# Nuttoty/Structured_Light_for_3D_Model_Replication

Hardware: AMD Instinct MI355X
Metric: decoded+triangulated px/s (higher is better)
Workload: dtype u8+f64

## Files before the change

structured_light_for_3d_model_replication_amd/csrc/slgpu.hip:

```cpp
#include <hip/hip_runtime.h>

#include <math.h>
#include <stdint.h>
#include <stdlib.h>
#include <string.h>

#include <stdio.h>

#include <algorithm>
#include <cmath>
#include <initializer_list>
#include <string>
#include <type_traits>
#include <thread>
#include <vector>

#include <dlfcn.h>
#include <errno.h>
#include <fcntl.h>
#include <sys/stat.h>
#include <unistd.h>

#include <chrono>
#include <condition_variable>
#include <memory>
#include <mutex>

#include "rccl/rccl.h"
#include "slgpu.h"

#pragma clang fp contract(off)

namespace {

constexpr int kThreads = 256;
constexpr int kWaves = kThreads / 64;
constexpr int kPx = 16;
constexpr int kChunk = 64 * kPx;
constexpr int kChunkNib = kChunk / 4;
constexpr int kRing = 40;
constexpr int kLoadAux = 2;
constexpr int kRecAux = 16;
constexpr int kMapAux = 2;
typedef unsigned v4u __attribute__((ext_vector_type(4)));
typedef unsigned v2u __attribute__((ext_vector_type(2)));
__device__ __forceinline__ uint4 ld_side16(const void* p) { return *reinterpret_cast<const uint4*>(p); }
__device__ __forceinline__ uint2 ld_side8(const void* p) { return *reinterpret_cast<const uint2*>(p); }
__device__ __forceinline__ uint32_t ld_side4(const void* p) { return *reinterpret_cast<const uint32_t*>(p); }

constexpr int M_MAPS = 1;
constexpr int M_CODES = 2;
constexpr int M_XYZ64 = 4;
constexpr int M_FROMMAPS = 8;
constexpr int M_NC = 16;
constexpr int M_ROWS = 32;
constexpr int M_HIST = 64;
constexpr int M_FAST32 = 128;
constexpr int M_PLANE_RSRC = 512;
constexpr int M_TEX = 2048;
constexpr int M_VERIFY = 4096;
constexpr int M_DECIDE = 256;
constexpr float kFastKappa = 16.0f;

constexpr int kSlot = 272;
constexpr int kSlotArrive = 257;
constexpr int kHistRep = 8;
constexpr int kHistStride = kHistRep + 1;
constexpr int kMaxWp = 32768;
constexpr int64_t kMaxChunks = 1 << 16;
constexpr int kRecSlot = 1536;

struct ViewStats {
  int thr_white;
  int thr_contrast;
  float noise_floor;
  float dynamic_range;
  unsigned pad[12];
};
static_assert(sizeof(ViewStats) % 64 == 0, "ViewStats keeps 64-B alignment");

struct Params {
  const uint8_t* stack;
  int64_t stack_vs;
  int view_bytes;
  const uint8_t* tex;
  int64_t tex_vs;
  const int32_t* in_col;
  const uint8_t* in_mask;
  int64_t HW;
  int H, W;
  uint32_t w_magic;
  int w_shift;
  int n_views;
  int cpv;
  int64_t n_chunks;
  int nc, nr, kc, kr;
  int mode;
  int Wp;
  const double4* planes;
  const float4* planes32;
  const double* xn;
  const double* yn;
  const float* xn32;
  const float* yn32;
  float fast_thr;
  int xy_safe;
  int xy_calc;
  double cx, cy, fx, fy;
  double rfx, rfy;
  const double* nc_rays;
  double o0, o1, o2;
  const double* poses;
  uint16_t* codes;
  int rec12;
  int rec_blk;
  uint8_t* ptnib;
  int32_t* col_out;
  int32_t* row_out;
  uint8_t* mask_out;
  void* xyz;
  uint8_t* bgr;
  int64_t out_cap;
  int64_t* view_offsets;
  ViewStats* stats;
  unsigned long long* masked;
  unsigned* hist;
  const int64_t* base_in;
  int* chunk_counts;
  int* block_sums;
  int bs_atomic;
  int decode_dyn;
  unsigned* super_base;
  unsigned* super_par;
  int sb_shift;
  int rerun;
  int cloud_gx;
  const uint8_t* pre_stack;
  int64_t pre_vs;
  unsigned* pre_hist;
  int pre_views;
  int pre_bpv;
};


__device__ __forceinline__ int64_t rec_slot(const Params& p, int view, int civ) {
  return (static_cast<int64_t>(civ >> 2) * p.n_views + view) * 4 + (civ & 3);
}

__device__ __forceinline__ uint4 ld16(const uint8_t* p, int n, bool vec) {
  if (vec) return *reinterpret_cast<const uint4*>(p);
  uint32_t w[4] = {0u, 0u, 0u, 0u};
#pragma unroll
  for (int i = 0; i < 16; ++i)
    if (i < n) w[i >> 2] |= static_cast<uint32_t>(p[i]) << (8 * (i & 3));
  return make_uint4(w[0], w[1], w[2], w[3]);
}

__device__ __forceinline__ uint32_t word(const uint4& q, int i) {
  return i == 0 ? q.x : i == 1 ? q.y : i == 2 ? q.z : q.w;
}

__device__ __forceinline__ uint32_t byte_of(const uint4& q, int i) {
// ... 175 lines not shown
  return fabs((pl.x * r0 + pl.y * r1) + pl.z * r2) > 1e-6;
}

__device__ __forceinline__ bool has_point(const Params& p, int mode, const float4& f, int c, float x, float y,
                                          float z, float inv, int u, int v, int64_t q) {
  const float a = fabsf((f.x * x + f.y * y + f.z * z) * inv);
  const float S = (fabsf(f.x * x) + fabsf(f.y * y) + fabsf(f.z * z)) * inv;
  const float B = S * 3.814697265625e-06f + 9.5367431640625e-13f;
  if (a > 1e-6f + B) return true;
  if (a < 1e-6f - B) return false;
  return has_point_f64(p.planes, p.xn, p.yn, (mode & M_NC) ? p.nc_rays : nullptr, p.HW, c, u, v, q);
}


__global__ __launch_bounds__(256) void k_xy_check(const double* xn, int W, const double* yn, int H, double cx,
                                                  double cy, double fx, double fy, int* bad) {
  const int i = static_cast<int>(blockIdx.x) * 256 + static_cast<int>(threadIdx.x);
  bool diff = false;
  if (i < W) diff = __double_as_longlong(xy_of(i, cx, fx)) != __double_as_longlong(xn[i]);
  else if (i < W + H) diff = __double_as_longlong(xy_of(i - W, cy, fy)) != __double_as_longlong(yn[i - W]);
  if (diff) *bad = 1;
}

constexpr int kHistRepl = 8;
constexpr int kHistView = kHistRepl * kSlot;

__device__ __forceinline__ void stats_pass(const uint8_t* vb, int64_t HW, int64_t blk, int64_t nblk, unsigned* gh,
                                           unsigned* s_hist, int* s_max) {
  const int tid = threadIdx.x;
  const int lane = tid & 63;
  const int wid = __builtin_amdgcn_readfirstlane(tid >> 6);
  for (int i = tid; i < 256 * kHistStride; i += kThreads) s_hist[i] = 0u;
  __syncthreads();
  unsigned* hrow = s_hist + (lane & (kHistRep - 1));
  int mx = -1024;
  const int64_t n16 = HW / 16;
  for (int64_t i = blk * kThreads + tid; i < n16; i += nblk * kThreads) {
    const uint4 wq = ld_side16(vb + 16 * i);
    const uint4 bq = ld_side16(vb + HW + 16 * i);
#pragma unroll
    for (int k = 0; k < 16; ++k) {
      const int bk = static_cast<int>(byte_of(bq, k));
      atomicAdd(hrow + bk * kHistStride, 1u);
      mx = max(mx, static_cast<int>(byte_of(wq, k)) - bk);
    }
  }
#pragma unroll
  for (int d = 32; d > 0; d >>= 1) mx = max(mx, __shfl_xor(mx, d, 64));
  if (lane == 0) s_max[wid] = mx;
  __syncthreads();
  gh += (blk % kHistRepl) * kSlot;
  unsigned cnt = 0u;
  const unsigned* row = s_hist + tid * kHistStride;
#pragma unroll
  for (int r = 0; r < kHistRep; ++r) cnt += row[r];
  if (cnt) atomicAdd(gh + tid, cnt);
  if (tid == 0) {
    int m = s_max[0];
#pragma unroll
    for (int w = 1; w < kWaves; ++w) m = max(m, s_max[w]);
    if (m > -1024) atomicMax(gh + 256, static_cast<unsigned>(m + 1024));
  }
}

__global__ __launch_bounds__(kThreads) void k_stats(Params p) {
  __shared__ unsigned s_hist[256 * kHistStride];
  __shared__ int s_max[kWaves];
  const int view = blockIdx.y;
  stats_pass(p.stack + view * p.stack_vs, p.HW, blockIdx.x, gridDim.x, p.hist + static_cast<int64_t>(view) * kHistView,
             s_hist, s_max);
}

__device__ __forceinline__ void pre_stats_block(const Params& p, int64_t sx, int64_t nsx, unsigned* s_hist,
                                                int* s_max) {
  const int64_t sblk = static_cast<int64_t>(blockIdx.y) * nsx + sx;
  const int64_t total = static_cast<int64_t>(p.pre_views) * p.pre_bpv;
  if (sblk < total) {
    const int pv = static_cast<int>(sblk / p.pre_bpv);
    stats_pass(p.pre_stack + pv * p.pre_vs, p.HW, sblk - static_cast<int64_t>(pv) * p.pre_bpv, p.pre_bpv,
               p.pre_hist + static_cast<int64_t>(pv) * kHistView, s_hist, s_max);
  }
}

__device__ __forceinline__ Thresholds view_thresholds(const Params& p, int view, int lane) {
  uint4 b4 = make_uint4(0u, 0u, 0u, 0u);
  unsigned hmax = 0u;
  const unsigned* h = p.hist + static_cast<int64_t>(view) * kHistView;
#pragma unroll
  for (int r = 0; r < kHistRepl; ++r) {
    const uint4 t = reinterpret_cast<const uint4*>(h + r * kSlot)[lane];
    b4.x += t.x;
    b4.y += t.y;
    b4.z += t.z;
    b4.w += t.w;
    hmax = max(hmax, h[r * kSlot + 256]);
  }
  return thresholds_from_bins(b4, hmax, p.HW, lane);
}

template <int S>
__device__ __forceinline__ bool arrive_last(unsigned* ctr, unsigned id, unsigned readers) {
  const unsigned cls = id & (S - 1);
  const unsigned n_cls = (readers - cls + S - 1) / S;
  if (atomicAdd(ctr + 1 + cls, 1u) + 1u != n_cls) return false;
  return atomicAdd(ctr, 1u) + 1u == min(readers, static_cast<unsigned>(S));
}

__device__ __forceinline__ void hist_release(unsigned* h, int words, unsigned id, unsigned readers, int lane,
                                             uint32_t dep0, uint32_t dep1) {
  asm volatile("" ::"v"(dep0), "v"(dep1) : "memory");
  unsigned last = 0u;
  if (lane == 0) last = arrive_last<8>(h + kSlotArrive, id, readers) ? 1u : 0u;
  if (__shfl(static_cast<int>(last), 0, 64)) {
    uint4* h4 = reinterpret_cast<uint4*>(h);
    for (int i = lane; i < words / 4; i += 64) h4[i] = make_uint4(0u, 0u, 0u, 0u);
  }
}

__device__ __forceinline__ uint32_t mask4(uint32_t w, uint32_t b, uint32_t tw2, uint32_t tc2, uint32_t* bytes) {
  const uint32_t we = w & 0x00ff00ffu, wo = (w >> 8) & 0x00ff00ffu;
  const uint32_t be = b & 0x00ff00ffu, bo = (b >> 8) & 0x00ff00ffu;
  const uint32_t me = ((we | 0x80008000u) - tw2) & (((we + 0x00100010u) | 0x80008000u) - (be + tc2));
  const uint32_t mo = ((wo | 0x80008000u) - tw2) & (((wo + 0x00100010u) | 0x80008000u) - (bo + tc2));
  const uint32_t y = ((me >> 15) & 0x00010001u) | ((mo >> 7) & 0x01000100u);
  *bytes = y;
  return (y & 1u) | ((y >> 7) & 2u) | ((y >> 14) & 4u) | ((y >> 21) & 8u);
}

constexpr int kDecPl = 2048, kDecX = 4096, kDecY = 4096;
constexpr int kDecPlWords = kDecPl * 4;
constexpr int kBsSlots = 64;
constexpr int kSuperCap = 4096;
constexpr int kSuperWords = 2 * kSuperCap + 4;

__device__ __forceinline__ unsigned* super_produce(const Params& p) {
  const unsigned sel = p.super_par[0] & 1u;
  if (!p.rerun && blockIdx.x == 0 && blockIdx.y == 0) {
    unsigned* other = p.super_base + (sel ^ 1u) * kSuperCap;
    for (int i = threadIdx.x; i < kSuperCap; i += kThreads) other[i] = 0u;
    if (threadIdx.x == 0) p.super_par[1] = sel;
  }
  return p.super_base + sel * kSuperCap;
}
__device__ __forceinline__ const unsigned* super_consume(const Params& p, int bx) {
  const unsigned sel = p.super_par[1] & 1u;
  if (!p.rerun && bx == 0 && blockIdx.y == 0 && threadIdx.x == 0) p.super_par[0] = sel ^ 1u;
  return p.super_base + sel * kSuperCap;
}
constexpr int kDecodeLds = (kDecPlWords + kDecX) * 4;
static_assert(kDecodeLds >= 256 * kHistStride * 4, "the decode LDS holds the histogram replicas too");

constexpr int kDecodePerCu = 3;
template <int KC, int KR, int MODE, int VEC>
__global__ __launch_bounds__(kThreads, 3) void k_decode(Params p) {
  const int mode = MODE >= 0 ? MODE : p.mode;
  const int kc = KC >= 0 ? KC : p.kc;
  const int krr = (mode & M_ROWS) ? (KR >= 0 ? KR : p.kr) : 0;
  const int nc = p.nc, nr = p.nr;
  const bool vec = VEC > 0;
  const bool hist = (mode & M_HIST) && !(mode & M_DECIDE);

  __shared__ __attribute__((aligned(16))) unsigned s_lds[kDecodeLds / 4];
  __shared__ int s_max[kWaves];
  __shared__ int s_cnt[2][kWaves];
  __shared__ unsigned s_bsum[kBsSlots];
  __shared__ uint32_t s_thr[2];
  __shared__ unsigned s_mcount;
  __shared__ int s_next[2];
  __shared__ uint4 s_mapst[(MODE < 0 || (MODE & M_MAPS)) ? 64 * kWaves : 1];
  unsigned* s_hist = s_lds;
  float4* s_pl = reinterpret_cast<float4*>(s_lds);
  float* s_xn = reinterpret_cast<float*>(s_lds) + kDecPlWords;
  const bool decide = (mode & M_DECIDE) != 0;
  const int tid = threadIdx.x;
  const int lane = tid & 63;
  const int wid = __builtin_amdgcn_readfirstlane(tid >> 6);
  const int view = blockIdx.y;
  const int64_t HW = p.HW;
  const int gx = static_cast<int>(gridDim.x);
  if (decide) {
    if (tid < kBsSlots) s_bsum[tid] = 0u;
    if (tid == 0) s_mcount = 0u;
    if ((mode & M_HIST) && wid == 0) {
      const Thresholds t = view_thresholds(p, view, lane);
      if (lane == 0) {
        s_thr[0] = static_cast<uint32_t>(t.white + 1) * 0x00010001u;
        s_thr[1] = static_cast<uint32_t>(t.contrast + 17) * 0x00010001u;
        if (blockIdx.x == 0) {
          p.stats[view].thr_white = t.white;
          p.stats[view].thr_contrast = t.contrast;
          p.stats[view].noise_floor = t.noise_floor;
          p.stats[view].dynamic_range = t.dynamic_range;
        }
      }
    }
    if (mode & M_CODES) {
      const int wp_t = min(p.Wp, kDecPl), w_t = min(p.W, kDecX);
      typedef __attribute__((address_space(3))) void* lds_ptr_t;
      for (int i = wid; i * 64 < wp_t; i += kWaves)
        __builtin_amdgcn_global_load_lds(p.planes32 + min(i * 64 + lane, wp_t - 1), (lds_ptr_t)(s_pl + i * 64), 16, 0, 0);
      for (int i = wid; i * 256 < w_t; i += kWaves)
        __builtin_amdgcn_global_load_lds(p.xn32 + min(i * 256 + 4 * lane, w_t - 4), (lds_ptr_t)(s_xn + i * 256), 16, 0, 0);
    }
  }
  uint32_t tw2 = static_cast<uint32_t>(40 + 1) * 0x00010001u;
  uint32_t tc2 = static_cast<uint32_t>(10 + 17) * 0x00010001u;
  int it = 0;

  if (hist) {
    for (int i = tid; i < 256 * kHistStride; i += kThreads) s_hist[i] = 0u;
    __syncthreads();
  }

  const int ngroups = (p.cpv + kWaves - 1) / kWaves;
  int mx_acc = -1024;
  const bool dyn = p.decode_dyn && decide && (mode & M_CODES) && !p.bs_atomic;
  unsigned* const sup = (decide && (mode & M_CODES)) ? super_produce(p) : nullptr;
  unsigned* const dyn_ctr = sup + (kSuperCap - 1 - view);
  for (int cg = blockIdx.x; cg < ngroups;) {
  unsigned dyn_next = 0u;
  if (dyn && tid == 0) dyn_next = atomicAdd(dyn_ctr, 1u);
  const int civ = cg * kWaves + wid;
  const bool live = civ < p.cpv;
  const int64_t px0 = static_cast<int64_t>(civ) * kChunk + lane * kPx;
  const int n_px = live ? static_cast<int>(min<int64_t>(max<int64_t>(HW - px0, 0), kPx)) : 0;
  const int64_t pxl = n_px > 0 ? px0 : 0;
  const int64_t o = view * HW + px0;

  const float ys_early = (decide && (mode & M_CODES) && n_px > 0) ? p.yn32[row_of(p, static_cast<int>(px0))] : 0.0f;
  uint32_t col[kPx];
  uint32_t pt_rec = 0xffffu;
  uint4 wq = make_uint4(0u, 0u, 0u, 0u), bq = wq;
  uint32_t rA[4] = {0, 0, 0, 0}, rB[4] = {0, 0, 0, 0};
  const int rBn = krr > 8 ? krr - 8 : 0;
  const int rSh = nr - krr;
  if (mode & M_FROMMAPS) {
    const int64_t ol = view * HW + pxl;
    if (vec) {
      const int4* cm = reinterpret_cast<const int4*>(p.in_col + ol);
#pragma unroll
      for (int i = 0; i < 4; ++i) {
        const int4 v = cm[i];
        col[4 * i] = static_cast<uint32_t>(max(v.x, 0));
        col[4 * i + 1] = static_cast<uint32_t>(max(v.y, 0));
        col[4 * i + 2] = static_cast<uint32_t>(max(v.z, 0));
        col[4 * i + 3] = static_cast<uint32_t>(max(v.w, 0));
      }
    } else {
#pragma unroll
      for (int k = 0; k < kPx; ++k) col[k] = k < n_px ? static_cast<uint32_t>(max(p.in_col[ol + k], 0)) : 0u;
    }
  } else {
    const uint8_t* vbase = p.stack + view * p.stack_vs;
    const int voff = static_cast<int>(pxl);
    const __amdgpu_buffer_rsrc_t rs_view =
        __builtin_amdgcn_make_buffer_rsrc(const_cast<uint8_t*>(vbase), 0, p.view_bytes, 0x00020000);
    auto ldp = [&](int plane) -> uint4 {
      if (vec && !(mode & M_PLANE_RSRC)) {
        const auto v = __builtin_amdgcn_raw_buffer_load_b128(rs_view, voff, plane * static_cast<int>(HW), kLoadAux);
        return make_uint4(v[0], v[1], v[2], v[3]);
      }
      if (vec) {
        const __amdgpu_buffer_rsrc_t rs = __builtin_amdgcn_make_buffer_rsrc(
            const_cast<uint8_t*>(vbase) + static_cast<int64_t>(plane) * HW, 0, static_cast<int>(HW), 0x00020000);
        const auto v = __builtin_amdgcn_raw_buffer_load_b128(rs, voff, 0, kLoadAux);
        return make_uint4(v[0], v[1], v[2], v[3]);
      }
      return ld16(vbase + pxl + static_cast<int64_t>(plane) * HW, n_px, false);
    };
    wq = ldp(0);
    bq = ldp(1);
    const int npl = 2 * (kc + krr);
    uint32_t cA[4] = {0, 0, 0, 0}, cB[4] = {0, 0, 0, 0};
    auto consume = [&](const uint4& P, const uint4& I, int pair) {
      auto ins = [](uint32_t acc, uint32_t g) { return ((acc >> 1) & 0x7f7f7f7fu) | (g & 0x80808080u); };
      uint32_t g[4];
#pragma unroll
      for (int w = 0; w < 4; ++w) g[w] = gt_bit7(word(P, w), word(I, w));
#pragma unroll
      for (int w = 0; w < 4; ++w) {
        if (pair < kc) {
          if (pair < 8) cA[w] = ins(cA[w], g[w]);
          else cB[w] = ins(cB[w], g[w]);
        } else if (pair - kc < 8) {
          rA[w] = ins(rA[w], g[w]);
        } else {
          rB[w] = ins(rB[w], g[w]);
        }
      }
// ... 32 lines not shown
            const uint4 I = ring[j + 1];
            if (pl + R < npl) {
              ring[j] = ldp(2 + pl + R);
              ring[j + 1] = ldp(3 + pl + R);
            }
            consume(P, I, pl >> 1);
          }
        }
      }
    }
    auto to_binary = [](uint32_t (&A)[4], uint32_t (&B)[4], int k) {
      const int kA = k < 8 ? k : 8, kB = k - kA;
#pragma unroll
      for (int w = 0; w < 4; ++w) {
        A[w] = gray_to_binary_bytes(__builtin_bitreverse32(A[w]), kA);
        B[w] = kB > 0 ? gray_to_binary_bytes(__builtin_bitreverse32(B[w]) ^ ((A[w] & 0x01010101u) << (kB - 1)), kB)
                      : 0u;
      }
    };
    const int cBn = kc > 8 ? kc - 8 : 0;
    const int cSh = nc - kc;
    to_binary(cA, cB, kc);
#pragma unroll
    for (int q = 0; q < kPx; ++q) {
      const int w = q >> 2, sft = 8 * (3 - (q & 3));
      col[q] = (((cA[w] >> sft) & 0xffu) << cBn) | ((cB[w] >> sft) & 0xffu);
    }
    if (cSh > 0) {
#pragma unroll
      for (int q = 0; q < kPx; ++q) {
        const uint32_t lo = col[q] & 1u;
        col[q] = (col[q] << cSh) | ((lo << cSh) - lo);
      }
    }
    if (mode & M_ROWS) to_binary(rA, rB, krr);
  }
  auto row_code = [&](int w, int e) -> uint32_t {
    const int sft = 8 * (3 - e);
    uint32_t v = (((rA[w] >> sft) & 0xffu) << rBn) | ((rB[w] >> sft) & 0xffu);
    if (rSh > 0) {
      const uint32_t lo = v & 1u;
      v = (v << rSh) | ((lo << rSh) - lo);
    }
    return v;
  };
  if (mode & M_MAPS) {
    if (vec && live) {
      uint4* const stg = s_mapst + 64 * wid;
      const int64_t cbase = view * HW + static_cast<int64_t>(civ) * kChunk;
#pragma unroll
      for (int m = 0; m < 2; ++m) {
        const __amdgpu_buffer_rsrc_t rd = __builtin_amdgcn_make_buffer_rsrc(
            (m == 0 ? p.col_out : p.row_out) + cbase, 0,
            static_cast<int>(4 * min<int64_t>(kChunk, HW - static_cast<int64_t>(civ) * kChunk)), 0x00020000);
#pragma unroll
        for (int j = 0; j < 4; ++j) {
          if ((lane >> 4) == j && n_px == kPx) {
            const int u = lane & 15;
#pragma unroll
            for (int q = 0; q < 4; ++q) {
              uint32_t v4[4];
#pragma unroll
              for (int e = 0; e < 4; ++e) v4[e] = m == 0 ? col[4 * q + e] : row_code(q, e);
              stg[4 * u + q] = make_uint4(v4[0], v4[1], v4[2], v4[3]);
            }
          }
          __builtin_amdgcn_wave_barrier();
          const uint4 v = stg[lane];
          __builtin_amdgcn_wave_barrier();
          __builtin_amdgcn_raw_buffer_store_b128(v4u{v.x, v.y, v.z, v.w}, rd, 1024 * j + 16 * lane, 0, kMapAux);
        }
      }
    } else if (!vec) {
#pragma unroll
      for (int k = 0; k < kPx; ++k) {
        if (k < n_px) {
          __builtin_nontemporal_store(static_cast<int32_t>(col[k]), p.col_out + o + k);
          __builtin_nontemporal_store(static_cast<int32_t>(row_code(k >> 2, k & 3)), p.row_out + o + k);
        }
      }
    }
  }
  if (decide) {
    if (it == 0) {
      __syncthreads();
      if (mode & M_HIST) {
        tw2 = __builtin_amdgcn_readfirstlane(s_thr[0]);
        tc2 = __builtin_amdgcn_readfirstlane(s_thr[1]);
      }
    }
    uint32_t ok = 0u, mb[4];
#pragma unroll
    for (int w = 0; w < 4; ++w) ok |= mask4(word(wq, w), word(bq, w), tw2, tc2, &mb[w]) << (4 * w);
    if (n_px != kPx) ok = 0u;
    if (p.masked) {
      const int mc = wave_sum_dpp(__popc(ok));
      if (lane == 0 && mc) atomicAdd(&s_mcount, static_cast<unsigned>(mc));
    }
    if ((mode & M_MAPS) && n_px == kPx)
      __builtin_nontemporal_store(v4u{mb[0], mb[1], mb[2], mb[3]}, reinterpret_cast<v4u*>(p.mask_out + o));
    uint32_t pt = 0u;
    if ((mode & M_CODES) && ok) {
      const int px0i = static_cast<int>(px0);
      const int v = row_of(p, px0i), u0 = px0i - v * p.W;
      float4 pf[kPx];
#pragma unroll
      for (int k = 0; k < kPx; ++k) pf[k] = s_pl[min(col[k], static_cast<uint32_t>(p.Wp - 1))];
      float xs[kPx];
#pragma unroll
      for (int q4 = 0; q4 < 4; ++q4) {
        const float4 x4 = reinterpret_cast<const float4*>(s_xn + u0)[q4];
        xs[4 * q4] = x4.x;
        xs[4 * q4 + 1] = x4.y;
        xs[4 * q4 + 2] = x4.z;
        xs[4 * q4 + 3] = x4.w;
      }
      const float ys = ys_early;
      uint32_t todo = ok;
      if (!(mode & M_NC)) {
#pragma unroll
        for (int k = 0; k < kPx; ++k) {
          const float a = fabsf(__builtin_fmaf(pf[k].x, xs[k], __builtin_fmaf(pf[k].y, ys, pf[k].z)));
          if (a > p.fast_thr) pt |= 1u << k;
        }
        pt &= ok;
        todo &= ~pt;
      }
#pragma unroll
      for (int k = 0; k < kPx; ++k) {
        if (!((todo >> k) & 1u)) continue;
        const int c = static_cast<int>(min(col[k], static_cast<uint32_t>(p.Wp - 1)));
        const int64_t q = px0 + k;
        float x, y, z, inv;
        if (mode & M_NC) {
          x = static_cast<float>(p.nc_rays[q]);
          y = static_cast<float>(p.nc_rays[HW + q]);
          z = static_cast<float>(p.nc_rays[2 * HW + q]);
          inv = 1.0f;
        } else {
          x = xs[k];
          y = ys;
          z = 1.0f;
          inv = __frsqrt_rn(x * x + y * y + 1.0f);
        }
        if (has_point(p, mode, pf[k], c, x, y, z, inv, u0 + k, v, q)) pt |= 1u << k;
      }
    }
    if (mode & M_CODES) {
      const int64_t gci = static_cast<int64_t>(view) * p.cpv + civ;
      pt_rec = pt;
      const int cnt = wave_sum_dpp(__popc(pt));
      if (lane == 0) {
        if (live) p.chunk_counts[gci] = cnt;
        const unsigned mine = live ? static_cast<unsigned>(cnt) : 0u;
        if (p.bs_atomic) {
          const unsigned old = atomicAdd(&s_bsum[it], (1u << 16) | mine);
          if ((old >> 16) == kWaves - 1) {
            const int64_t blk = static_cast<int64_t>(view) * ngroups + cg;
            const unsigned t = (old & 0xffffu) + mine;
            p.block_sums[blk] = static_cast<int>(t);
            if (t) atomicAdd(sup + (blk >> p.sb_shift), t);
          }
        } else {
          s_cnt[it & 1][wid] = static_cast<int>(mine);
        }
      }
    }
  }
  if (hist) {
    unsigned* hrow = s_hist + (lane & (kHistRep - 1));
    int mx = -1024;
#pragma unroll
    for (int k = 0; k < kPx; ++k) {
      if (k < n_px) {
        const int bk = static_cast<int>(byte_of(bq, k));
        atomicAdd(hrow + bk * kHistStride, 1u);
        mx = max(mx, static_cast<int>(byte_of(wq, k)) - bk);
      }
    }
    mx_acc = max(mx_acc, mx);
  }

  if (mode & M_CODES) {
    uint32_t rec[kPx / 2];
#pragma unroll
    for (int i = 0; i < kPx / 2; ++i)
      rec[i] = min(col[2 * i], static_cast<uint32_t>(p.Wp - 1)) |
               (min(col[2 * i + 1], static_cast<uint32_t>(p.Wp - 1)) << 16);
    if (decide) {
      const bool blk = !(mode & M_MAPS);
      if (n_px == kPx) {
        uint32_t rw[6];
        uint32_t* ro = blk ? rw : reinterpret_cast<uint32_t*>(reinterpret_cast<uint8_t*>(p.codes) + 3 * o / 2);
#pragma unroll
        for (int h = 0; h < 2; ++h) {
          const uint32_t* r = rec + 4 * h;
          auto cd = [&](int k, uint32_t c) { return ((pt_rec >> (8 * h + k)) & 1u) ? c : 0xfffu; };
          const uint32_t c0 = cd(0, r[0] & 0xffffu), c1 = cd(1, r[0] >> 16), c2 = cd(2, r[1] & 0xffffu);
          const uint32_t c3 = cd(3, r[1] >> 16), c4 = cd(4, r[2] & 0xffffu), c5 = cd(5, r[2] >> 16);
          const uint32_t c6 = cd(6, r[3] & 0xffffu), c7 = cd(7, r[3] >> 16);
          ro[3 * h] = c0 | (c1 << 12) | (c2 << 24);
          ro[3 * h + 1] = (c2 >> 8) | (c3 << 4) | (c4 << 16) | (c5 << 28);
          ro[3 * h + 2] = (c5 >> 4) | (c6 << 8) | (c7 << 20);
        }
        if (blk) {
          const __amdgpu_buffer_rsrc_t rs = __builtin_amdgcn_make_buffer_rsrc(
              reinterpret_cast<uint8_t*>(p.codes) + kRecSlot * rec_slot(p, view, civ), 0, kRecSlot, 0x00020000);
          __builtin_amdgcn_raw_buffer_store_b128(v4u{rw[0], rw[1], rw[2], rw[3]}, rs, 16 * lane, 0, kRecAux);
          __builtin_amdgcn_raw_buffer_store_b64(v2u{rw[4], rw[5]}, rs, 1024 + 8 * lane, 0, kRecAux);
        }
      }
    } else if (vec) {
      if (n_px == kPx) {
        uint4* ro = reinterpret_cast<uint4*>(p.codes + o);
        ro[0] = make_uint4(rec[0], rec[1], rec[2], rec[3]);
        ro[1] = make_uint4(rec[4], rec[5], rec[6], rec[7]);
      }
    } else {
#pragma unroll
      for (int k = 0; k < kPx; ++k)
        if (k < n_px) p.codes[o + k] = static_cast<uint16_t>(rec[k >> 1] >> (16 * (k & 1)));
    }
  }
  if (decide && (mode & M_CODES) && !p.bs_atomic) {
    if (dyn && tid == 0) s_next[it & 1] = static_cast<int>(dyn_next) + gx;
    __syncthreads();
    if (tid == 0) {
      int t = 0;
#pragma unroll
      for (int w = 0; w < kWaves; ++w) t += s_cnt[it & 1][w];
      const int64_t blk = static_cast<int64_t>(view) * ngroups + cg;
      p.block_sums[blk] = t;
      if (t) atomicAdd(sup + (blk >> p.sb_shift), static_cast<unsigned>(t));
    }
  }
  cg = dyn ? s_next[it & 1] : cg + gx;
  ++it;
  }

  if (decide && p.masked) {
    __syncthreads();
    if (tid == 0 && s_mcount) atomicAdd(p.masked + view, static_cast<unsigned long long>(s_mcount));
  }
  if (decide && (mode & M_HIST) && !p.rerun && wid == 0)
    hist_release(p.hist + static_cast<int64_t>(view) * kHistView, kHistView, blockIdx.x, gx, lane, tw2, tc2);

  if (hist) {
#pragma unroll
    for (int d = 32; d > 0; d >>= 1) mx_acc = max(mx_acc, __shfl_xor(mx_acc, d, 64));
    if (lane == 0) s_max[wid] = mx_acc;
    __syncthreads();
    unsigned* gh = p.hist + view * kSlot;
    unsigned cnt = 0u;
    const unsigned* row = s_hist + tid * kHistStride;
#pragma unroll
    for (int r = 0; r < kHistRep; ++r) cnt += row[r];
    if (cnt) atomicAdd(gh + tid, cnt);
    if (tid == 0) {
      int m = s_max[0];
#pragma unroll
      for (int w = 1; w < kWaves; ++w) m = max(m, s_max[w]);
      if (m > -1024) atomicMax(gh + 256, static_cast<unsigned>(m + 1024));
    }
  }
}

template <int VEC>
__device__ __forceinline__ int count_chunk(const Params& p, int64_t gc, int view, int civ, int lane, bool live,
                                           int* masked) {
  const int mode = p.mode;
  const bool vec = VEC > 0;
  const int HW = static_cast<int>(p.HW);
  const int cpx = civ * kChunk;
  const int W = p.W;
  const bool codes = (mode & M_CODES) != 0;
  const bool nc = (mode & M_NC) != 0;
  const uint8_t* vstack = p.stack + view * p.stack_vs;
  const uint16_t* vcodes = codes ? p.codes + static_cast<int64_t>(view) * HW : nullptr;

  uint4 hb = make_uint4(0u, 0u, 0u, 0u);
  unsigned hmax = 0u;
  const bool adaptive = (mode & M_HIST) != 0;
  if (adaptive) {
    const unsigned* h = p.hist + view * kSlot;
    hb = reinterpret_cast<const uint4*>(h)[lane];
    hmax = h[256];
  }
  uint32_t wv[4], bv[4];
  uint32_t rc[4][2];
  const int px_hi = vec ? HW - 4 : HW - 1;
#pragma unroll
  for (int s = 0; s < 4; ++s) {
    const int px = min(cpx + 256 * s + 4 * lane, px_hi);
    if (mode & M_FROMMAPS) {
      wv[s] = bv[s] = 0u;
    } else if (vec) {
      wv[s] = ld_side4(vstack + px);
      bv[s] = ld_side4(vstack + HW + px);
    } else {
      uint32_t a = 0u, b = 0u;
#pragma unroll
      for (int e = 0; e < 4; ++e) {
        const int q = min(px + e, HW - 1);
        a |= static_cast<uint32_t>(vstack[q]) << (8 * e);
        b |= static_cast<uint32_t>(vstack[HW + q]) << (8 * e);
      }
      wv[s] = a;
      bv[s] = b;
    }
    if (codes) {
      if (vec) {
        const uint2 r = ld_side8(vcodes + px);
        rc[s][0] = r.x;
        rc[s][1] = r.y;
      } else {
        rc[s][0] = vcodes[min(px, HW - 1)] | (static_cast<uint32_t>(vcodes[min(px + 1, HW - 1)]) << 16);
        rc[s][1] = vcodes[min(px + 2, HW - 1)] | (static_cast<uint32_t>(vcodes[min(px + 3, HW - 1)]) << 16);
      }
    }
  }
  uint32_t mk[4] = {0u, 0u, 0u, 0u};
  if (mode & M_FROMMAPS) {
    const uint8_t* vm = p.in_mask + static_cast<int64_t>(view) * HW;
#pragma unroll
    for (int s = 0; s < 4; ++s) {
      const int px = cpx + 256 * s + 4 * lane;
#pragma unroll
      for (int e = 0; e < 4; ++e) mk[s] |= (px + e < HW && vm[px + e] != 0) ? (1u << e) : 0u;
    }
// ... 986 lines not shown
}

__global__ __launch_bounds__(256) void k_zero(unsigned* p, int64_t n) {
  for (int64_t i = static_cast<int64_t>(blockIdx.x) * 256 + threadIdx.x; i < n; i += 256ll * gridDim.x) p[i] = 0u;
}
int zero_async(sl_ctx* c, void* p, int64_t words, hipStream_t s) {
  if (words <= 0) return SL_OK;
  const unsigned blocks = static_cast<unsigned>(std::min<int64_t>((words + 255) / 256, 1024));
  hipLaunchKernelGGL(k_zero, dim3(blocks), dim3(256), 0, s, static_cast<unsigned*>(p), words);
  HIP_TRY(c, hipGetLastError());
  return SL_OK;
}
int capture_of(sl_ctx* c, hipStream_t s, unsigned long long* out) {
  hipStreamCaptureStatus st = hipStreamCaptureStatusNone;
  unsigned long long id = 0;
  HIP_TRY(c, hipStreamGetCaptureInfo(s, &st, &id));
  *out = st == hipStreamCaptureStatusActive ? id + 1 : 0;
  return SL_OK;
}

int launch_groups(sl_ctx* c, const Params& p0, bool vec, int decode_mode, int count_mode, int cloud_mode,
                  hipStream_t s, PreArms arms) {
  const bool decide = (decode_mode & M_DECIDE) != 0;
  const bool codes = (decode_mode & M_CODES) != 0;
  const int64_t cpv = p0.cpv;
  const int vpg = static_cast<int>(std::max<int64_t>(1, kMaxChunks / cpv));
  const int n_groups = static_cast<int>((p0.n_views + vpg - 1) / vpg);
  const bool adaptive = (decode_mode & M_HIST) != 0;
  const bool pre_run = arms.decl && cloud_mode >= 0 && vec;
  bool hist_fresh = false;
  int r = ensure_scratch(c, std::min(vpg, p0.n_views), p0.HW, codes, pre_run ? std::min(vpg, c->decl_views) : 0,
                         &hist_fresh, s, true);
  if (r) return r;
  r = grow(c, &c->d_stats, &c->cap_stats, p0.n_views, s, true);
  if (r) return r;
  unsigned long long cap_id = 0;
  r = capture_of(c, s, &cap_id);
  if (r) return r;
  const int nv0 = std::min(vpg, p0.n_views);
  const bool pre_use = arms.armed && !hist_fresh && decide && adaptive && p0.stack == c->pre_stack &&
                       p0.stack_vs == c->pre_vs && nv0 == c->pre_views && p0.HW == c->pre_hw &&
                       c->pre_capture == cap_id;
  const bool pre_groups = decide && adaptive && n_groups > 1 && cloud_mode >= 0 && vec;
  const int dom = cap_id ? 1 : 0;
  unsigned* const hbuf = c->d_hist[dom];
  int64_t& hist_dirty = c->hist_dirty[dom];
  if (dom == 1 && c->cap_domain != cap_id) {
    c->cap_domain = cap_id;
    hist_dirty = c->cap_hist;
  }
  if (c->super_dirty) {
    r = zero_async(c, c->d_super, kSuperWords, s);
    if (r) return r;
  }
  c->super_dirty = false;
  if (!pre_use && hist_dirty > 0) {
    r = zero_async(c, hbuf, hist_dirty, s);
    if (r) return r;
  }
  if (!pre_use) hist_dirty = 0;
  auto pre_bpv_of = [&](int nv) -> int64_t {
    const int64_t per_view = (p0.HW / 16 + kThreads - 1) / kThreads;
    return std::max<int64_t>(1, std::min<int64_t>(per_view, (c->pre_wgs + nv - 1) / nv));
  };
  c->last_views = p0.n_views;
  if (p0.masked) {
    r = zero_async(c, p0.masked, 2 * static_cast<int64_t>(p0.n_views), s);
    if (r) return r;
  }
  hipEvent_t* ev = nullptr;
  if (!c->prof_ev.empty() && kProfEv * (c->prof_n + 1) <= static_cast<int>(c->prof_ev.size()))
    ev = &c->prof_ev[kProfEv * c->prof_n++];
  auto add_pre = [&](Params& pc, dim3& grid, int nv, const uint8_t* pst, int64_t pvs, int pnv) {
    const int64_t bpv = pre_bpv_of(pnv);
    pc.pre_stack = pst;
    pc.pre_vs = pvs;
    pc.pre_hist = hbuf;
    pc.pre_views = pnv;
    pc.pre_bpv = static_cast<int>(bpv);
    const int64_t total = static_cast<int64_t>(pnv) * bpv;
    grid.x += static_cast<unsigned>((total + nv - 1) / nv);
    hist_dirty = static_cast<int64_t>(pnv) * kHistView;
  };
  bool next_pre = pre_use;
  int g = 0;
  for (int v0 = 0; v0 < p0.n_views; v0 += vpg, ++g) {
    hipEvent_t* gev = (ev && g < kProfGroups) ? ev + 4 * g : nullptr;
    if (gev) HIP_TRY(c, hipEventRecord(gev[0], s));
    const int nv = std::min(vpg, p0.n_views - v0);
    c->last_launch_px = static_cast<int64_t>(nv) * p0.HW;
    Params p = p0;
    p.n_views = nv;
    p.n_chunks = static_cast<int64_t>(nv) * cpv;
    if (p.stack) p.stack += v0 * p.stack_vs;
    if (p.tex) p.tex += v0 * p.tex_vs;
    if (p.in_col) p.in_col += v0 * p.HW;
    if (p.in_mask) p.in_mask += v0 * p.HW;
    if (p.col_out) p.col_out += v0 * p.HW;
    if (p.row_out) p.row_out += v0 * p.HW;
    if (p.mask_out) p.mask_out += v0 * p.HW;
    if (p.poses) p.poses += 16 * v0;
    if (p.masked) p.masked += v0;
    if (p.view_offsets) p.view_offsets += v0;
    p.base_in = (v0 > 0 && p.view_offsets) ? p.view_offsets : nullptr;
    p.stats = c->d_stats + v0;
    p.codes = c->d_codes;
    p.rec12 = (decide && cloud_mode >= 0) ? 1 : 0;
    p.rec_blk = (p.rec12 && !(decode_mode & M_MAPS)) ? 1 : 0;
    p.ptnib = c->d_ptnib;
    p.chunk_counts = c->d_chunk_counts;
    p.block_sums = c->d_block_sums;
    p.hist = hbuf;
    p.super_base = c->d_super;
    p.super_par = c->d_super + 2 * kSuperCap;
    const bool pre_g = next_pre;
    next_pre = false;
    const dim3 grid(static_cast<unsigned>((cpv + kWaves - 1) / kWaves), static_cast<unsigned>(nv));
    {
      const int64_t nb = static_cast<int64_t>(grid.x) * nv;
      int sh = 0;
      while ((int64_t{1} << (2 * sh)) < nb) ++sh;
      p.sb_shift = sh;
    }
    c->last.valid = true;
    dim3 dgrid = grid;
    if (c->decode_wgs > 0) dgrid.x = std::min(grid.x, static_cast<unsigned>(std::max(1, (c->decode_wgs + nv - 1) / nv)));
    c->last.grid[0] = dgrid;
    p.bs_atomic = decide && (grid.x + dgrid.x - 1) / dgrid.x <= static_cast<unsigned>(kBsSlots);
    p.decode_dyn = (!(decode_mode & M_MAPS) && decide && codes && dgrid.x < grid.x &&
                    ((static_cast<int64_t>(grid.x) * nv) >> p.sb_shift) + 1 + nv < kSuperCap) ? 1 : 0;
    if (p.decode_dyn) p.bs_atomic = 0;
    c->last.grid[1] = c->last.grid[2] = grid;
    c->last.s = s;
    c->last.fn[1] = c->last.fn[2] = nullptr;
    c->last.decide = decide;
    c->last.stats = false;
    if (decide) {
      if (adaptive) {
        const int64_t per_view = (p0.HW / 16 + kThreads - 1) / kThreads;
        const dim3 sg(static_cast<unsigned>(std::max<int64_t>(1, std::min<int64_t>(per_view, (2 * c->n_cu + nv - 1) / nv))),
                      static_cast<unsigned>(nv));
        p.mode = decode_mode;
        c->last.p[1] = p;
        c->last.grid[1] = sg;
        c->last.stats = true;
        if (!pre_g) {
          void* args[] = {&p};
          const void* kst = reinterpret_cast<const void*>(k_stats);
          c->last.fn[1] = kst;
          HIP_TRY(c, hipLaunchKernel(kst, sg, dim3(kThreads), args, 0, s));
        }
      }
      if (gev) HIP_TRY(c, hipEventRecord(gev[1], s));
    }
    if (codes) c->super_dirty = true;
    {
      p.mode = decode_mode;
      KernelFn fn = pick_decode(p.kc, (decode_mode & M_ROWS) ? p.kr : 0, decode_mode, vec);
      c->last.p[0] = p;
      c->last.p[0].masked = nullptr;
      c->last.fn[0] = reinterpret_cast<const void*>(fn);
      void* args[] = {&p};
      HIP_TRY(c, hipLaunchKernel(reinterpret_cast<const void*>(fn), dgrid, dim3(kThreads), args, 0, s));
      hist_dirty = (adaptive && !decide) ? static_cast<int64_t>(nv) * kSlot : 0;
    }
    if (gev) HIP_TRY(c, hipEventRecord(gev[decide ? 2 : 1], s));
    if (!decide) {
      p.mode = count_mode;
      void* args[] = {&p};
      const void* fn = vec ? reinterpret_cast<const void*>(k_count<1>) : reinterpret_cast<const void*>(k_count<0>);
      c->last.p[1] = p;
      c->last.p[1].masked = nullptr;
      c->last.fn[1] = fn;
      HIP_TRY(c, hipLaunchKernel(fn, grid, dim3(kThreads), args, 0, s));
      hist_dirty = 0;
    }
    if (gev && !decide) HIP_TRY(c, hipEventRecord(gev[2], s));
    if (cloud_mode >= 0) {
      p.mode = cloud_mode;
      p.cloud_gx = static_cast<int>(grid.x);
      KernelFn fn = pick_cloud(cloud_mode, vec);
      c->last.p[2] = p;
      c->last.fn[2] = reinterpret_cast<const void*>(fn);
      Params pc = p;
      dim3 cgrid = grid;
      const bool last_g = g == n_groups - 1;
      const bool pre_now = pre_run && last_g;
      const bool pre_grp = pre_groups && !last_g;
      if (pre_now)
        add_pre(pc, cgrid, nv, c->decl_stack, c->decl_vs, std::min(vpg, c->decl_views));
      else if (pre_grp)
        add_pre(pc, cgrid, nv, p0.stack + static_cast<int64_t>(v0 + vpg) * p0.stack_vs, p0.stack_vs,
                std::min(vpg, p0.n_views - v0 - vpg));
      void* args[] = {&pc};
      HIP_TRY(c, hipLaunchKernel(reinterpret_cast<const void*>(fn), cgrid, dim3(kThreads), args, 0, s));
      c->super_dirty = false;
      if (pre_now) {
        c->pre_armed = true;
        c->pre_stack = c->decl_stack;
        c->pre_vs = c->decl_vs;
        c->pre_views = std::min(vpg, c->decl_views);
        c->pre_hw = p0.HW;
        c->pre_capture = cap_id;
      }
      next_pre = pre_grp;
    }
    if (gev) HIP_TRY(c, hipEventRecord(gev[3], s));
  }
  if (ev) {
    c->prof_groups.push_back(std::min(g, kProfGroups));
    c->prof_decide.push_back(decide);
  }
  c->last_launches = g;
  return SL_OK;
}

int launch(sl_ctx* c, const Params& p0, bool vec, int decode_mode, int count_mode, int cloud_mode, hipStream_t s,
           PreArms arms) {
  const int r = launch_groups(c, p0, vec, decode_mode, count_mode, cloud_mode, s, arms);
  if (r) {
    c->hist_dirty[0] = c->hist_dirty[1] = c->cap_hist;
    c->super_dirty = c->d_super != nullptr;
    c->pre_armed = false;
  }
  return r;
}

int stream_handoff(sl_ctx* c, hipStream_t s) {
  if (c->done_valid && s != c->last_stream) {
    HIP_TRY(c, hipEventRecord(c->done_ev, c->last_stream));
    HIP_TRY(c, hipStreamWaitEvent(s, c->done_ev, 0));
  }
  c->last_stream = s;
  c->done_valid = true;
  return SL_OK;
}

}

int slgpu_fail(sl_ctx* c, int code, const char* msg) { return fail(c, code, msg); }
int slgpu_device(const sl_ctx* c) { return c->device; }

namespace {

__host__ __device__ inline bool fmt4_exact(double x) {
  return __builtin_isfinite(x) && __builtin_fabs(x) < 9.0e11;
}

__host__ __device__ inline uint64_t fmt4_scaled(double x, bool* neg) {
  const uint64_t bits = static_cast<uint64_t>(__builtin_bit_cast(int64_t, x));
  *neg = bits >> 63;
  const int be = static_cast<int>((bits >> 52) & 0x7ff);
  const uint64_t frac = bits & ((1ull << 52) - 1);
  const uint64_t m = be ? (frac | (1ull << 52)) : frac;
  const int e = (be ? be : 1) - 1075;
  unsigned __int128 v = static_cast<unsigned __int128>(m) * 10000u;
  uint64_t N;
  if (e >= 0) {
    N = static_cast<uint64_t>(v << e);
  } else if (-e >= 120) {
    N = 0;
  } else {
    const int sh = -e;
    const unsigned __int128 q = v >> sh;
    const unsigned __int128 r = v - (q << sh);
    const unsigned __int128 half = static_cast<unsigned __int128>(1) << (sh - 1);
    N = static_cast<uint64_t>(q);
    if (r > half || (r == half && (N & 1u))) ++N;
  }
  return N;
}

__host__ __device__ inline int fmt4_len(double x) {
  bool neg;
  uint64_t ip = fmt4_scaled(x, &neg) / 10000u;
  int d = 1;
  while (ip >= 10u) {
    ip /= 10u;
    ++d;
// ... 719 lines not shown
    return fail(c, SL_EINVAL, "sl_mask_counts_to: counts must be 8-byte aligned");
  c->mc_next = device_counts;
  return SL_OK;
}

int sl_sync(sl_ctx* c, void* stream) {
  if (!c) return SL_EINVAL;
  HIP_TRY(c, hipSetDevice(c->device));
  HIP_TRY(c, hipStreamSynchronize(static_cast<hipStream_t>(stream)));
  HIP_TRY(c, hipGetLastError());
  return SL_OK;
}

int sl_profile_enable(sl_ctx* c, int max_calls) {
  if (!c || max_calls < 0) return SL_EINVAL;
  HIP_TRY(c, hipSetDevice(c->device));
  for (hipEvent_t e : c->prof_ev) HIP_TRY(c, hipEventDestroy(e));
  c->prof_ev.clear();
  c->prof_groups.clear();
  c->prof_decide.clear();
  c->prof_n = 0;
  for (int i = 0; i < kProfEv * max_calls; ++i) {
    hipEvent_t e;
    HIP_TRY(c, hipEventCreate(&e));
    c->prof_ev.push_back(e);
  }
  return SL_OK;
}

int sl_profile_read(sl_ctx* c, double* decode_ms, double* count_ms, double* cloud_ms, int* calls) {
  if (!c) return SL_EINVAL;
  HIP_TRY(c, hipSetDevice(c->device));
  double t[3] = {0.0, 0.0, 0.0};
  for (int i = 0; i < c->prof_n; ++i) {
    const int ng = i < static_cast<int>(c->prof_groups.size()) ? c->prof_groups[i] : 0;
    for (int g = 0; g < ng; ++g) {
      hipEvent_t* ev = &c->prof_ev[kProfEv * i + 4 * g];
      HIP_TRY(c, hipEventSynchronize(ev[3]));
      const bool dz = i < static_cast<int>(c->prof_decide.size()) && c->prof_decide[i];
      for (int k = 0; k < 3; ++k) {
        float ms = 0.f;
        HIP_TRY(c, hipEventElapsedTime(&ms, ev[k], ev[k + 1]));
        t[dz ? (k == 0 ? 1 : k == 1 ? 0 : 2) : k] += ms;
      }
    }
  }
  c->prof_groups.clear();
  c->prof_decide.clear();
  if (decode_ms) *decode_ms = t[0];
  if (count_ms) *count_ms = t[1];
  if (cloud_ms) *cloud_ms = t[2];
  if (calls) *calls = c->prof_n;
  c->prof_n = 0;
  return SL_OK;
}

int sl_time_kernels(sl_ctx* c, int reps, double* decode_ms, double* count_ms, double* cloud_ms) {
  if (!c || reps < 1) return SL_EINVAL;
  if (!c->last.valid) return fail(c, SL_EINVAL, "sl_time_kernels: no earlier call to re-run");
  HIP_TRY(c, hipSetDevice(c->device));
  hipStream_t s = c->last.s;
  {
    hipStreamCaptureStatus st = hipStreamCaptureStatusNone;
    HIP_TRY(c, hipStreamIsCapturing(s, &st));
    if (st != hipStreamCaptureStatusNone)
      return fail(c, SL_EINVAL, "sl_time_kernels: the last call's stream is capturing (re-runs are eager only)");
  }
  Params pr[3];
  for (int k = 0; k < 3; ++k) {
    pr[k] = c->last.p[k];
    pr[k].rerun = 1;
  }
  auto run = [&](const void* fn, int k) -> hipError_t {
    Params q = pr[k];
    void* args[] = {&q};
    return hipLaunchKernel(fn, c->last.grid[k], dim3(kThreads), args, 0, s);
  };
  auto clear = [&]() -> hipError_t {
    hipError_t e = hipMemsetAsync(c->d_hist[0], 0, sizeof(unsigned) * c->cap_hist, s);
    if (e == hipSuccess) e = hipMemsetAsync(c->d_hist[1], 0, sizeof(unsigned) * c->cap_hist, s);
    if (e == hipSuccess) e = hipMemsetAsync(c->d_super, 0, sizeof(unsigned) * kSuperWords, s);
    return e;
  };
  hipError_t e = clear();
  if (e == hipSuccess && c->last.decide && c->last.stats) e = run(reinterpret_cast<const void*>(k_stats), 1);
  if (e == hipSuccess) e = run(c->last.fn[0], 0);
  if (e == hipSuccess && !c->last.decide && c->last.fn[1]) e = run(c->last.fn[1], 1);
  hipEvent_t ev[4] = {nullptr, nullptr, nullptr, nullptr};
  for (int k = 0; k < 4 && e == hipSuccess; ++k) e = hipEventCreate(&ev[k]);
  int r = e == hipSuccess ? SL_OK : fail(c, SL_EHIP, std::string("sl_time_kernels: ") + hipGetErrorString(e));
  const int order3[3] = {2, 1, 0}, orderd[3] = {2, 0, 1};
  const int* order = c->last.decide ? orderd : order3;
  if (r == SL_OK && hipEventRecord(ev[0], s) != hipSuccess) r = fail(c, SL_EHIP, "hipEventRecord");
  for (int q = 0; q < 3 && r == SL_OK; ++q) {
    const int k = order[q];
    if (c->last.fn[k]) {
      for (int i = 0; i < reps; ++i) {
        e = run(c->last.fn[k], k);
        if (e != hipSuccess) {
          r = fail(c, SL_EHIP, std::string("sl_time_kernels: ") + hipGetErrorString(e));
          break;
        }
      }
    }
    if (r == SL_OK && hipEventRecord(ev[q + 1], s) != hipSuccess) r = fail(c, SL_EHIP, "hipEventRecord");
  }
  double out[3] = {0.0, 0.0, 0.0};
  if (r == SL_OK && hipEventSynchronize(ev[3]) == hipSuccess) {
    for (int q = 0; q < 3; ++q) {
      float ms = 0.f;
      const int k = order[q];
      if (hipEventElapsedTime(&ms, ev[q], ev[q + 1]) == hipSuccess) out[k] = c->last.fn[k] ? ms / reps : 0.0;
    }
  }
  if (r == SL_OK && c->last.fn[0] && c->last.p[0].decode_dyn) {
    const unsigned nv = c->last.grid[0].y;
    unsigned* ctr = c->d_super + (kSuperCap - nv);
    double sum = 0.0;
    for (int i = 0; i < reps && r == SL_OK; ++i) {
      float ms = 0.f;
      if (hipMemsetAsync(ctr, 0, sizeof(unsigned) * nv, s) != hipSuccess || hipEventRecord(ev[0], s) != hipSuccess ||
          run(c->last.fn[0], 0) != hipSuccess || hipEventRecord(ev[1], s) != hipSuccess ||
          hipEventSynchronize(ev[1]) != hipSuccess || hipEventElapsedTime(&ms, ev[0], ev[1]) != hipSuccess) {
        r = fail(c, SL_EHIP, "sl_time_kernels: dynamic k_decode re-run");
        break;
      }
      sum += ms;
    }
    if (r == SL_OK) out[0] = sum / reps;
  }
  for (int k = 0; k < 4; ++k)
    if (ev[k]) (void)hipEventDestroy(ev[k]);
  if (clear() != hipSuccess && r == SL_OK) r = fail(c, SL_EHIP, "sl_time_kernels: scratch reset");
  c->hist_dirty[0] = c->hist_dirty[1] = 0;
  c->super_dirty = r != SL_OK;
  c->pre_armed = false;
  c->last.valid = false;
  if (decode_ms) *decode_ms = out[0];
  if (count_ms) *count_ms = out[1];
  if (cloud_ms) *cloud_ms = out[2];
  return r;
}

int sl_last_launch_info(sl_ctx* c, int* path, int64_t* launches, int64_t* last_launch_px) {
  if (!c) return SL_EINVAL;
  if (path) *path = c->last.decide ? 1 : 0;
  if (launches) *launches = c->last_launches;
  if (last_launch_px) *last_launch_px = c->last_launch_px;
  return SL_OK;
}

int sl_last_thresholds(sl_ctx* c, int view, float* nf, float* dr, int* thr_w, int* thr_c) {
  if (!c) return SL_EINVAL;
  if (view < 0 || view >= c->last_views || !c->d_stats) return fail(c, SL_EINVAL, "no such view");
  HIP_TRY(c, hipSetDevice(c->device));
  HIP_TRY(c, hipDeviceSynchronize());
  ViewStats s;
  HIP_TRY(c, hipMemcpy(&s, c->d_stats + view, sizeof(ViewStats), hipMemcpyDeviceToHost));
  if (nf) *nf = s.noise_floor;
  if (dr) *dr = s.dynamic_range;
  if (thr_w) *thr_w = s.thr_white;
  if (thr_c) *thr_c = s.thr_contrast;
  return SL_OK;
}

int sl_format_ply(const void* xyz, int xyz_dtype, const uint8_t* bgr, int64_t n, int threads, char* out,
                  int64_t out_capacity, int64_t* out_len) {
  if (!out_len || !ply_args_ok(xyz, xyz_dtype, bgr, n)) return SL_EINVAL;
  std::lock_guard<std::mutex> lk(ply_mutex());
  PlyParts parts;
  ply_format(xyz, xyz_dtype, bgr, n, threads, parts);
  int64_t len = static_cast<int64_t>(parts.head.size());
  for (size_t l : parts.len) len += static_cast<int64_t>(l);
  *out_len = len;
  if (!out) return SL_OK;
  if (out_capacity < len) return SL_ECAPACITY;
  memcpy(out, parts.head.data(), parts.head.size());
  int64_t off = static_cast<int64_t>(parts.head.size());
  for (size_t t = 0; t < parts.len.size(); ++t) {
    if (parts.len[t]) memcpy(out + off, parts.ptr[t], parts.len[t]);
    off += static_cast<int64_t>(parts.len[t]);
  }
  return SL_OK;
}

int sl_write_ply(const char* path, const void* xyz, int xyz_dtype, const uint8_t* bgr, int64_t n, int threads) {
  if (!path || !ply_args_ok(xyz, xyz_dtype, bgr, n)) return SL_EINVAL;
  std::lock_guard<std::mutex> lk(ply_mutex());
  PlyParts parts;
// ... 283 lines not shown
```

Before: 80.16 billion.

## Compute per-view thresholds once in a separate kernel instead of per decode block

Adds a small k_thresholds kernel that reduces the histogram replicas into thresholds once per view, writes a 16-byte record into histogram padding, and clears the histogram. Decode blocks now read that record directly instead of each wave-0 recomputing thresholds from the replicas. This also removes the in-kernel arrive-last histogram release and the shared-memory broadcast. The cost is one extra kernel launch per group and a serialization point between stats and decode.

```diff
diff --git a/structured_light_for_3d_model_replication_amd/csrc/slgpu.hip b/structured_light_for_3d_model_replication_amd/csrc/slgpu.hip
--- a/structured_light_for_3d_model_replication_amd/csrc/slgpu.hip
+++ b/structured_light_for_3d_model_replication_amd/csrc/slgpu.hip
@@ -78,6 +78,12 @@
   unsigned pad[12];
 };
 static_assert(sizeof(ViewStats) % 64 == 0, "ViewStats keeps 64-B alignment");
+
+struct __attribute__((aligned(16))) ThrRecord {
+  int thr_white, thr_contrast;
+  float noise_floor, dynamic_range;
+};
+static_assert(sizeof(ThrRecord) == 16, "one 16-byte load per workgroup");
 
 struct Params {
   const uint8_t* stack;
@@ -419,10 +425,17 @@
   }
 }
 
-__device__ __forceinline__ Thresholds view_thresholds(const Params& p, int view, int lane) {
+constexpr int kThrWord = kSlot - 4;
+static_assert(kThrWord >= kSlotArrive + 9 && kThrWord % 4 == 0 && kHistView % 4 == 0, "the record is 16 pad bytes, aligned");
+__device__ __forceinline__ ThrRecord* thr_record(unsigned* hist, int view) {
+  return reinterpret_cast<ThrRecord*>(hist + static_cast<int64_t>(view) * kHistView + kThrWord);
+}
+__global__ __launch_bounds__(64) void k_thresholds(unsigned* hist, int64_t n) {
+  const int view = blockIdx.x;
+  const int lane = threadIdx.x;
+  unsigned* h = hist + static_cast<int64_t>(view) * kHistView;
   uint4 b4 = make_uint4(0u, 0u, 0u, 0u);
   unsigned hmax = 0u;
-  const unsigned* h = p.hist + static_cast<int64_t>(view) * kHistView;
 #pragma unroll
   for (int r = 0; r < kHistRepl; ++r) {
     const uint4 t = reinterpret_cast<const uint4*>(h + r * kSlot)[lane];
@@ -432,7 +445,19 @@
     b4.w += t.w;
     hmax = max(hmax, h[r * kSlot + 256]);
   }
-  return thresholds_from_bins(b4, hmax, p.HW, lane);
+  const Thresholds t = thresholds_from_bins(b4, hmax, n, lane);
+  if (lane == 0) {
+    ThrRecord o;
+    o.thr_white = t.white;
+    o.thr_contrast = t.contrast;
+    o.noise_floor = t.noise_floor;
+    o.dynamic_range = t.dynamic_range;
+    *thr_record(hist, view) = o;
+  }
+  asm volatile("" ::"v"(t.white), "v"(t.contrast) : "memory");
+  uint4* h4 = reinterpret_cast<uint4*>(h);
+  for (int i = lane; i < kHistView / 4; i += 64)
+    if (i != kThrWord / 4) h4[i] = make_uint4(0u, 0u, 0u, 0u);
 }
 
 template <int S>
@@ -501,7 +526,6 @@
   __shared__ int s_max[kWaves];
   __shared__ int s_cnt[2][kWaves];
   __shared__ unsigned s_bsum[kBsSlots];
-  __shared__ uint32_t s_thr[2];
   __shared__ unsigned s_mcount;
   __shared__ int s_next[2];
   __shared__ uint4 s_mapst[(MODE < 0 || (MODE & M_MAPS)) ? 64 * kWaves : 1];
@@ -515,22 +539,22 @@
   const int view = blockIdx.y;
   const int64_t HW = p.HW;
   const int gx = static_cast<int>(gridDim.x);
+  uint32_t tw2 = static_cast<uint32_t>(40 + 1) * 0x00010001u;
+  uint32_t tc2 = static_cast<uint32_t>(10 + 17) * 0x00010001u;
   if (decide) {
+    if (mode & M_HIST) {
+      const ThrRecord t = *thr_record(p.hist, view);
+      tw2 = static_cast<uint32_t>(t.thr_white + 1) * 0x00010001u;
+      tc2 = static_cast<uint32_t>(t.thr_contrast + 17) * 0x00010001u;
+      if (blockIdx.x == 0 && tid == 0) {
+        p.stats[view].thr_white = t.thr_white;
+        p.stats[view].thr_contrast = t.thr_contrast;
+        p.stats[view].noise_floor = t.noise_floor;
+        p.stats[view].dynamic_range = t.dynamic_range;
+      }
+    }
     if (tid < kBsSlots) s_bsum[tid] = 0u;
     if (tid == 0) s_mcount = 0u;
-    if ((mode & M_HIST) && wid == 0) {
-      const Thresholds t = view_thresholds(p, view, lane);
-      if (lane == 0) {
-        s_thr[0] = static_cast<uint32_t>(t.white + 1) * 0x00010001u;
-        s_thr[1] = static_cast<uint32_t>(t.contrast + 17) * 0x00010001u;
-        if (blockIdx.x == 0) {
-          p.stats[view].thr_white = t.white;
-          p.stats[view].thr_contrast = t.contrast;
-          p.stats[view].noise_floor = t.noise_floor;
-          p.stats[view].dynamic_range = t.dynamic_range;
-        }
-      }
-    }
     if (mode & M_CODES) {
       const int wp_t = min(p.Wp, kDecPl), w_t = min(p.W, kDecX);
       typedef __attribute__((address_space(3))) void* lds_ptr_t;
@@ -540,8 +564,6 @@
         __builtin_amdgcn_global_load_lds(p.xn32 + min(i * 256 + 4 * lane, w_t - 4), (lds_ptr_t)(s_xn + i * 256), 16, 0, 0);
     }
   }
-  uint32_t tw2 = static_cast<uint32_t>(40 + 1) * 0x00010001u;
-  uint32_t tc2 = static_cast<uint32_t>(10 + 17) * 0x00010001u;
   int it = 0;
 
   if (hist) {
@@ -740,13 +762,7 @@
     }
   }
   if (decide) {
-    if (it == 0) {
-      __syncthreads();
-      if (mode & M_HIST) {
-        tw2 = __builtin_amdgcn_readfirstlane(s_thr[0]);
-        tc2 = __builtin_amdgcn_readfirstlane(s_thr[1]);
-      }
-    }
+    if (it == 0) __syncthreads();
     uint32_t ok = 0u, mb[4];
 #pragma unroll
     for (int w = 0; w < 4; ++w) ok |= mask4(word(wq, w), word(bq, w), tw2, tc2, &mb[w]) << (4 * w);
@@ -900,9 +916,6 @@
     __syncthreads();
     if (tid == 0 && s_mcount) atomicAdd(p.masked + view, static_cast<unsigned long long>(s_mcount));
   }
-  if (decide && (mode & M_HIST) && !p.rerun && wid == 0)
-    hist_release(p.hist + static_cast<int64_t>(view) * kHistView, kHistView, blockIdx.x, gx, lane, tw2, tc2);
-
   if (hist) {
 #pragma unroll
     for (int d = 32; d > 0; d >>= 1) mx_acc = max(mx_acc, __shfl_xor(mx_acc, d, 64));
@@ -2055,6 +2068,12 @@
     grid.x += static_cast<unsigned>((total + nv - 1) / nv);
     hist_dirty = static_cast<int64_t>(pnv) * kHistView;
   };
+  auto thresholds = [&](int nv) -> int {
+    hipLaunchKernelGGL(k_thresholds, dim3(static_cast<unsigned>(nv)), dim3(64), 0, s, hbuf, p0.HW);
+    HIP_TRY(c, hipGetLastError());
+    hist_dirty = 0;
+    return SL_OK;
+  };
   bool next_pre = pre_use;
   int g = 0;
   for (int v0 = 0; v0 < p0.n_views; v0 += vpg, ++g) {
@@ -2121,7 +2140,10 @@
           void* args[] = {&p};
           const void* kst = reinterpret_cast<const void*>(k_stats);
           c->last.fn[1] = kst;
+          hist_dirty = static_cast<int64_t>(nv) * kHistView;
           HIP_TRY(c, hipLaunchKernel(kst, sg, dim3(kThreads), args, 0, s));
+          r = thresholds(nv);
+          if (r) return r;
         }
       }
       if (gev) HIP_TRY(c, hipEventRecord(gev[1], s));
@@ -2168,6 +2190,10 @@
       void* args[] = {&pc};
       HIP_TRY(c, hipLaunchKernel(reinterpret_cast<const void*>(fn), cgrid, dim3(kThreads), args, 0, s));
       c->super_dirty = false;
+      if (pre_now || pre_grp) {
+        r = thresholds(pc.pre_views);
+        if (r) return r;
+      }
       if (pre_now) {
         c->pre_armed = true;
         c->pre_stack = c->decl_stack;
@@ -3053,8 +3079,15 @@
     if (e == hipSuccess) e = hipMemsetAsync(c->d_super, 0, sizeof(unsigned) * kSuperWords, s);
     return e;
   };
+  const bool restats = c->last.decide && c->last.stats;
+  auto thresholds = [&]() -> hipError_t {
+    const Params& q = pr[1];
+    hipLaunchKernelGGL(k_thresholds, dim3(c->last.grid[1].y), dim3(64), 0, s, q.hist, q.HW);
+    return hipGetLastError();
+  };
   hipError_t e = clear();
-  if (e == hipSuccess && c->last.decide && c->last.stats) e = run(reinterpret_cast<const void*>(k_stats), 1);
+  if (e == hipSuccess && restats) e = run(reinterpret_cast<const void*>(k_stats), 1);
+  if (e == hipSuccess && restats) e = thresholds();
   if (e == hipSuccess) e = run(c->last.fn[0], 0);
   if (e == hipSuccess && !c->last.decide && c->last.fn[1]) e = run(c->last.fn[1], 1);
   hipEvent_t ev[4] = {nullptr, nullptr, nullptr, nullptr};
@@ -3076,6 +3109,8 @@
     }
     if (r == SL_OK && hipEventRecord(ev[q + 1], s) != hipSuccess) r = fail(c, SL_EHIP, "hipEventRecord");
   }
+  if (r == SL_OK && restats && c->last.fn[1] && thresholds() != hipSuccess)
+    r = fail(c, SL_EHIP, "sl_time_kernels: k_thresholds");
   double out[3] = {0.0, 0.0, 0.0};
   if (r == SL_OK && hipEventSynchronize(ev[3]) == hipSuccess) {
     for (int q = 0; q < 3; ++q) {
```

Result: slower. 78.71 billion (-1.8%).
